# kvas7andy/unreal

Hardware: AMD Instinct MI355X
Metric: env-steps/sec (whole node), UNREAL maze 84x84 (higher is better)
Workload: dtype f32 (fp16x2-split MFMA operands, fp32 accumulate)

## Files before the change

unreal_amd/csrc/pc.hip:

```cpp
#include "common.h"

namespace {

constexpr int HP_LD = 36, HP_ROWS = 84;
constexpr int NPLP = 2;
constexpr int WD_ELEMS = 4 * 4 * 2 * 4 * 16 * 4;
constexpr int HP_V = (C2_POS * 8 + 255) / 256;
constexpr int DD_V = (PC_CELLS * 8 / 4 + 255) / 256;

struct PcFwdArgs {
  int N, A;
  const float* hp;
  const float* hp_absmax;
  const float* Wv; const float* bv; const float* Wa; const float* ba;
  float* qmax;
  const int* action;
  const float* target;
  const int* mask;
  float lambda, grad_scale;
  float* d_dec;
  float* ddec_absmax;
  float* loss;
};

__device__ __forceinline__ float deconv_w(const float* __restrict__ Wv, const float* __restrict__ Wa, int A, int ky, int kx,
                                          int co, int ci) {
  if (co == 0) return Wv[(ky * 4 + kx) * 32 + ci];
  if (co <= A) return Wa[((ky * 4 + kx) * A + (co - 1)) * 32 + ci];
  return 0.f;
}

__device__ __forceinline__ void hp_load(const float* __restrict__ src, int gtid, f32x4 (&r)[HP_V]) {
  const f32x4* s4 = reinterpret_cast<const f32x4*>(src);
#pragma unroll
  for (int c = 0; c < HP_V; ++c) {
    int id = gtid + 256 * c;
    r[c] = s4[id < C2_POS * 8 ? id : gtid];
  }
}

__device__ __forceinline__ void hp_store(float* hp, int gtid, const f32x4 (&r)[HP_V]) {
#pragma unroll
  for (int c = 0; c < HP_V; ++c) {
    int id = gtid + 256 * c;
    if (id < C2_POS * 8) *reinterpret_cast<f32x4*>(hp + (id >> 3) * HP_LD + (id & 7) * 4) = r[c];
  }
}

typedef _Float16 fh8p __attribute__((ext_vector_type(8)));
typedef _Float16 fh2p __attribute__((ext_vector_type(2)));
typedef float f32x2p __attribute__((ext_vector_type(2)));
typedef unsigned int u32x2p __attribute__((ext_vector_type(2)));

constexpr int HPP_ROW = 80;
constexpr int HPP_PLANE = HP_ROWS * HPP_ROW;
constexpr int WDP_ROW = 80;
constexpr int WDP_PLANE = 4 * 32 * WDP_ROW;

__device__ __forceinline__ void split4p(const f32x4& v, float scale, u32x2p (&pl)[NPLP]) {
  const f32x2p x01 = (f32x2p){v[0], v[1]} * scale, x23 = (f32x2p){v[2], v[3]} * scale;
  const fh2p h01 = __builtin_convertvector(x01, fh2p), h23 = __builtin_convertvector(x23, fh2p);
  const fh2p l01 = __builtin_convertvector(x01 - __builtin_convertvector(h01, f32x2p), fh2p);
  const fh2p l23 = __builtin_convertvector(x23 - __builtin_convertvector(h23, f32x2p), fh2p);
  pl[0] = (u32x2p){__builtin_bit_cast(unsigned int, h01), __builtin_bit_cast(unsigned int, h23)};
  pl[1] = (u32x2p){__builtin_bit_cast(unsigned int, l01), __builtin_bit_cast(unsigned int, l23)};
}

__device__ __forceinline__ void hp_store_planes(unsigned char* hpp, int gtid, const f32x4 (&r)[HP_V], float scale) {
#pragma unroll
  for (int c = 0; c < HP_V; ++c) {
    const int id = gtid + 256 * c;
    if (id < C2_POS * 8) {
      u32x2p pl[NPLP];
      split4p(r[c], scale, pl);
      pl[0][0] = keep_positive_visible(pl[0][0], r[c][0], r[c][1]);
      pl[0][1] = keep_positive_visible(pl[0][1], r[c][2], r[c][3]);
#pragma unroll
      for (int t = 0; t < NPLP; ++t) *reinterpret_cast<u32x2p*>(hpp + t * HPP_PLANE + (id >> 3) * HPP_ROW + (id & 7) * 8) = pl[t];
    }
  }
}

#define PC_MFMA(a, b, c) __builtin_amdgcn_mfma_f32_16x16x32_f16((a), (b), (c), 0, 0, 0)
#define PC_SPLIT_MMA(A, B, C)        \
  do {                               \
    C = PC_MFMA(A[1], B[0], C);      \
    C = PC_MFMA(A[0], B[1], C);      \
    C = PC_MFMA(A[0], B[0], C);      \
  } while (0)

__device__ __forceinline__ float pc_weight_max(const float* __restrict__ Wv, const float* __restrict__ Wa, int A, float* red) {
  if (threadIdx.x == 0) *red = 0.f;
  __syncthreads();
  float m = 0.f;
  for (int e = threadIdx.x; e < 512; e += 256) m = fmaxf(m, fabsf(Wv[e]));
  for (int e = threadIdx.x; e < 512 * A; e += 256) m = fmaxf(m, fabsf(Wa[e]));
  m = wave_max(m);
  if ((threadIdx.x & 63) == 0) atomicMax(reinterpret_cast<unsigned int*>(red), __float_as_uint(m));
  __syncthreads();
  return *red;
}

__device__ __forceinline__ void pc_fwd_weight_planes(const float* __restrict__ Wv, const float* __restrict__ Wa, int A,
                                                     unsigned char* wdp, float S_W) {
  const int CO = 1 + A;
  for (int e = threadIdx.x; e < 4 * 32 * 8; e += 256) {
    const int c4 = e & 7, n = (e >> 3) & 31, dd = e >> 8;
    f32x4 v = {0.f, 0.f, 0.f, 0.f};
    if (n < 4 * CO) {
      const int par = n / CO, co = n - par * CO;
      const int ky = (par >> 1) + 2 * (dd >> 1), kx = (par & 1) + 2 * (dd & 1);
#pragma unroll
      for (int k = 0; k < 4; ++k) v[k] = deconv_w(Wv, Wa, A, ky, kx, co, 4 * c4 + k);
    }
    u32x2p pl[NPLP];
    split4p(v, S_W, pl);
#pragma unroll
    for (int t = 0; t < NPLP; ++t) *reinterpret_cast<u32x2p*>(wdp + t * WDP_PLANE + (dd * 32 + n) * WDP_ROW + c4 * 8) = pl[t];
  }
}

__device__ __forceinline__ void pc_zero_hp_pad_rows(unsigned char* hpp) {
  for (int e = threadIdx.x; e < NPLP * 3 * HPP_ROW / 4; e += 256) {
    const int t = e / (3 * HPP_ROW / 4), w = e % (3 * HPP_ROW / 4);
    reinterpret_cast<uint32_t*>(hpp + t * HPP_PLANE + C2_POS * HPP_ROW)[w] = 0u;
  }
}

template <int COT> struct FwdLds {
  static constexpr int DS = COT | 1;
  static constexpr int DEC = NPLP * HPP_PLANE, DOUT = DEC + PC_CELLS * DS * 4, W = DOUT + PC_CELLS * COT * 4,
                       BYTES = W + NPLP * WDP_PLANE;
  static constexpr int WGS = 3 * BYTES <= 160 * 1024 ? 3 : 2;
};

template <bool TWO_NT, int DS>
__device__ __forceinline__ void deconv_packed(const unsigned char* hpp, const unsigned char* wdp, float* dec, int mt0, int i,
                                              int q, int CO, const float (&bias)[2], float unscale) {
  constexpr int NTL = TWO_NT ? 2 : 1;
  const int ntiles = (mt0 + 4 < 7) ? 2 : 1;
  f32x4 acc[2][NTL];
  int a[2], b[2];
#pragma unroll
  for (int t = 0; t < 2; ++t) {
#pragma unroll
    for (int nt = 0; nt < NTL; ++nt) acc[t][nt] = (f32x4){0.f, 0.f, 0.f, 0.f};
    const int m = min((mt0 + 4 * t) * 16 + i, 99);
    a[t] = m / 10;
    b[t] = m % 10;
  }
#pragma unroll
  for (int dd = 0; dd < 4; ++dd) {
    const int da = dd >> 1, db = dd & 1;
    fh8p bw[NTL][NPLP];
#pragma unroll
    for (int nt = 0; nt < NTL; ++nt)
#pragma unroll
      for (int pl = 0; pl < NPLP; ++pl)
        bw[nt][pl] = *reinterpret_cast<const fh8p*>(wdp + pl * WDP_PLANE + ((dd * 32 + nt * 16 + i)) * WDP_ROW + 16 * q);
#pragma unroll
    for (int t = 0; t < 2; ++t) {
      if (t < ntiles) {
        const int y = a[t] - da, x = b[t] - db;
        const int row = (y >= 0 && y < 9 && x >= 0 && x < 9) ? y * 9 + x : C2_POS;
        fh8p av[NPLP];
#pragma unroll
        for (int pl = 0; pl < NPLP; ++pl)
          av[pl] = *reinterpret_cast<const fh8p*>(hpp + pl * HPP_PLANE + row * HPP_ROW + 16 * q);
#pragma unroll
        for (int nt = 0; nt < NTL; ++nt) PC_SPLIT_MMA(av, bw[nt], acc[t][nt]);
      }
    }
  }
#pragma unroll
  for (int nt = 0; nt < NTL; ++nt) {
    const int n = nt * 16 + i;
    if (n < 4 * CO) {
      const int par = n / CO, co = n - par * CO;
#pragma unroll
      for (int t = 0; t < 2; ++t)
        if (t < ntiles) {
#pragma unroll
          for (int r = 0; r < 4; ++r) {
            const int m = (mt0 + 4 * t) * 16 + 4 * q + r;
            if (m < 100)
              dec[((2 * (m / 10) + (par >> 1)) * 20 + 2 * (m % 10) + (par & 1)) * DS + co] = acc[t][nt][r] * unscale + bias[nt];
          }
        }
    }
  }
}

template <int COT>
__global__ __launch_bounds__(256, FwdLds<COT>::WGS) void pc_deconv_fwd_kernel(PcFwdArgs p) {
  typedef FwdLds<COT> L;
  constexpr int DS = L::DS;
  __shared__ __attribute__((aligned(16))) unsigned char smem[L::BYTES];
  __shared__ float s_red;
  const int gtid = threadIdx.x;
  const int lane = threadIdx.x & 63, gw = gtid >> 6;
  const int i = lane & 15, q = lane >> 4;
  unsigned char* hpp = smem;
  float* dec = reinterpret_cast<float*>(smem + L::DEC);
  float* dout = reinterpret_cast<float*>(smem + L::DOUT);
  unsigned char* wdp = smem + L::W;
  const int A = p.A, CO = 1 + p.A;

  const float S_W = pow2_scale(pc_weight_max(p.Wv, p.Wa, A, &s_red));
  const float S_HP = pow2_scale(*p.hp_absmax);
  const float unscale = pow2_inv(S_HP) * pow2_inv(S_W);

  pc_fwd_weight_planes(p.Wv, p.Wa, A, wdp, S_W);
  pc_zero_hp_pad_rows(hpp);
  float bias[2];
#pragma unroll
  for (int nt = 0; nt < 2; ++nt) {
    const int n = nt * 16 + i;
    const int co = n % CO;
    bias[nt] = (n < 4 * CO) ? (co == 0 ? p.bv[0] : p.ba[co - 1]) : 0.f;
  }
  const bool two_nt = 4 * CO > 16;
  float loss_acc = 0.f, dd_max = 0.f;

  const int stride = gridDim.x;
  f32x4 pre[HP_V];
  {
    const int n0 = blockIdx.x;
    if (n0 < p.N) {
      hp_load(p.hp + (size_t)n0 * F2_DIM, gtid, pre);
      hp_store_planes(hpp, gtid, pre, S_HP);
    }
  }
  int prev = -1;
  for (int base = blockIdx.x; base < p.N; base += stride) {
    const int n = base;
    const bool valid = n < p.N;
    const int nn = n + stride;
    const bool has_next = nn < p.N;
    __syncthreads();
    if (prev >= 0 && p.d_dec) {
      f32x4* dst = reinterpret_cast<f32x4*>(p.d_dec + (size_t)prev * PC_CELLS * CO);
      for (int id = gtid; id < PC_CELLS * CO / 4; id += 256) dst[id] = reinterpret_cast<const f32x4*>(dout)[id];
    }
    if (has_next) hp_load(p.hp + (size_t)nn * F2_DIM, gtid, pre);
    float tg[2] = {0.f, 0.f};
    int act = 0;
    bool on = true;
    if (valid && p.d_dec) {
      tg[0] = p.target[(size_t)n * PC_CELLS + gtid];
      tg[1] = p.target[(size_t)n * PC_CELLS + min(gtid + 256, PC_CELLS - 1)];
      act = p.action[n];
      on = p.mask[n] != 0;
    }
    if (valid) {
      if (two_nt) deconv_packed<true, DS>(hpp, wdp, dec, gw, i, q, CO, bias, unscale);
      else deconv_packed<false, DS>(hpp, wdp, dec, gw, i, q, CO, bias, unscale);
    }
    __syncthreads();
    if (valid) {
#pragma unroll
      for (int pi = 0; pi < 2; ++pi) {
        const int pos = gtid + 256 * pi;
        if (pos >= PC_CELLS) break;
        const float* d = dec + pos * DS;
        const float vpre = d[0];
        const float V = fmaxf(vpre, 0.f);
        float adv[8], mean = 0.f;
        for (int k = 0; k < A; ++k) { adv[k] = fmaxf(d[1 + k], 0.f); mean += adv[k]; }
        mean /= (float)A;
        if (p.qmax) {
          float mx = V + adv[0] - mean;
          for (int k = 1; k < A; ++k) mx = fmaxf(mx, V + adv[k] - mean);
          p.qmax[(size_t)n * PC_CELLS + pos] = mx;
        }
        if (p.d_dec) {
          const float qa = V + adv[act] - mean;
          const float diff = tg[pi] - qa;
          const float dq = on ? -p.lambda * diff * p.grad_scale : 0.f;
          if (on) loss_acc += 0.5f * p.lambda * diff * diff;
          float* o = dout + pos * CO;
          o[0] = vpre > 0.f ? dq : 0.f;
          dd_max = fmaxf(dd_max, fabsf(dq));
          for (int k = 0; k < A; ++k)
            o[1 + k] = d[1 + k] > 0.f ? dq * (((k == act) ? 1.f : 0.f) - 1.f / (float)A) : 0.f;
        }
      }
    }
    if (has_next) hp_store_planes(hpp, gtid, pre, S_HP);
    prev = valid ? n : -1;
  }
  __syncthreads();
  if (prev >= 0 && p.d_dec) {
    f32x4* dst = reinterpret_cast<f32x4*>(p.d_dec + (size_t)prev * PC_CELLS * CO);
    for (int id = gtid; id < PC_CELLS * CO / 4; id += 256) dst[id] = reinterpret_cast<const f32x4*>(dout)[id];
  }
  {
    __shared__ float wsum[4], wmx[4];
    loss_acc = wave_sum(loss_acc);
    dd_max = wave_max(dd_max);
    if (lane == 0) { wsum[gw] = loss_acc; wmx[gw] = dd_max; }
    __syncthreads();
    if (gw == 0) {
      if (p.loss && lane == 0) atomicAdd(p.loss, (((wsum[0] + wsum[1]) + wsum[2]) + wsum[3]) * p.grad_scale);
      if (p.ddec_absmax) absmax_commit(p.ddec_absmax, fmaxf(fmaxf(wmx[0], wmx[1]), fmaxf(wmx[2], wmx[3])));
    }
  }
}

struct PcBwdArgs {
  int N, A;
  const float* hp;
  const float* hp_absmax;
  const float* d_dec;
  const float* ddec_absmax;
  const float* Wv; const float* Wa;
  float* d_hp;
  float* dWv; float* dbv; float* dWa; float* dba;
  float* dhp_absmax;
};

typedef short s16x4p __attribute__((ext_vector_type(4)));
typedef short s16x8p __attribute__((ext_vector_type(8)));
constexpr int DDP_ROW = 16;
constexpr int DDP_PLANE = (PC_CELLS + 4) * DDP_ROW;
constexpr int WBP_PLANE = 4 * 32 * WDP_ROW;
constexpr int BWD_GRP_BYTES = NPLP * HPP_PLANE + NPLP * DDP_PLANE + F2_DIM * 4;

__device__ __forceinline__ fh8p tr_pair_p(const unsigned char* a0, const unsigned char* a1) {
  typedef s16x4p __attribute__((address_space(3))) * lds_p;
  const s16x4p lo = __builtin_amdgcn_ds_read_tr16_b64_v4i16((lds_p)(a0));
  const s16x4p hi = __builtin_amdgcn_ds_read_tr16_b64_v4i16((lds_p)(a1));
  const s16x8p v = __builtin_shufflevector(lo, hi, 0, 1, 2, 3, 4, 5, 6, 7);
  return __builtin_bit_cast(fh8p, v);
}

__device__ __forceinline__ void split1p(float x, float scale, unsigned short (&t)[NPLP]) {
  x *= scale;
  const _Float16 h = (_Float16)x;
  const _Float16 l = (_Float16)(x - (float)h);
  t[0] = __builtin_bit_cast(unsigned short, h);
  t[1] = __builtin_bit_cast(unsigned short, l);
}

__device__ __forceinline__ void pc_bwd_weight_planes(const float* __restrict__ Wv, const float* __restrict__ Wa, int A,
                                                     unsigned char* wbp, float S_W) {
  for (int e = threadIdx.x; e < 4 * 32 * 32; e += 256) {
    const int k = e & 31, ci = (e >> 5) & 31, ky = e >> 10;
    const int kx = k >> 3, co = k & 7;
    float v = 0.f;
    if (co == 0) v = Wv[(ky * 4 + kx) * 32 + ci];
    else if (co <= A) v = Wa[((ky * 4 + kx) * A + (co - 1)) * 32 + ci];
    unsigned short t[NPLP];
    split1p(v, S_W, t);
#pragma unroll
    for (int pl = 0; pl < NPLP; ++pl)
      reinterpret_cast<unsigned short*>(wbp + pl * WBP_PLANE + (ky * 32 + ci) * WDP_ROW)[k] = t[pl];
  }
}

__device__ __forceinline__ void pc_stage_dd(unsigned char* ddp, int gtid, const float (&dd)[2][8], float S_DD, float (&adbk)[8]) {
#pragma unroll
  for (int h = 0; h < 2; ++h) {
    const int pos = gtid + 256 * h;
    if (pos < PC_CELLS) {
      u32x2p lo[NPLP], hi[NPLP];
      split4p((f32x4){dd[h][0], dd[h][1], dd[h][2], dd[h][3]}, S_DD, lo);
      split4p((f32x4){dd[h][4], dd[h][5], dd[h][6], dd[h][7]}, S_DD, hi);
#pragma unroll
      for (int pl = 0; pl < NPLP; ++pl) {
        typedef unsigned int u32x4p __attribute__((ext_vector_type(4)));
        *reinterpret_cast<u32x4p*>(ddp + pl * DDP_PLANE + pos * DDP_ROW) = (u32x4p){lo[pl][0], lo[pl][1], hi[pl][0], hi[pl][1]};
      }
#pragma unroll
      for (int k = 0; k < 8; ++k) adbk[k] += dd[h][k];
    }
  }
}

__device__ __forceinline__ void pc_dgrad_frame(const unsigned char* hpp, const unsigned char* ddp, const unsigned char* wbp,
                                               float* dhs, int gw, int i, int q, float un_dgrad) {
  const int nt = gw & 1;
  f32x4 acc[3];
  int abase[3];
#pragma unroll
  for (int jj = 0; jj < 3; ++jj) {
    acc[jj] = (f32x4){0.f, 0.f, 0.f, 0.f};
    const int pos = min(((gw >> 1) + 2 * jj) * 16 + i, C2_POS - 1);
    abase[jj] = ((2 * (pos / 9)) * 20 + 2 * (pos % 9) + q) * DDP_ROW;
  }
#pragma unroll
  for (int ky = 0; ky < 4; ++ky) {
    fh8p bw[NPLP];
#pragma unroll
    for (int pl = 0; pl < NPLP; ++pl)
      bw[pl] = *reinterpret_cast<const fh8p*>(wbp + pl * WBP_PLANE + (ky * 32 + nt * 16 + i) * WDP_ROW + 16 * q);
#pragma unroll
    for (int jj = 0; jj < 3; ++jj) {
      fh8p av[NPLP];
#pragma unroll
      for (int pl = 0; pl < NPLP; ++pl)
        av[pl] = *reinterpret_cast<const fh8p*>(ddp + pl * DDP_PLANE + abase[jj] + ky * 20 * DDP_ROW);
      PC_SPLIT_MMA(av, bw, acc[jj]);
    }
  }
#pragma unroll
  for (int jj = 0; jj < 3; ++jj)
#pragma unroll
    for (int r = 0; r < 4; ++r) {
      const int pos = ((gw >> 1) + 2 * jj) * 16 + 4 * q + r;
      if (pos < C2_POS) {
        const int ci = nt * 16 + i;
        const unsigned short h0 = reinterpret_cast<const unsigned short*>(hpp + pos * HPP_ROW)[ci];
        dhs[pos * 32 + ci] = (h0 != 0 && !(h0 & 0x8000)) ? acc[jj][r] * un_dgrad : 0.f;
      }
    }
}

__device__ __forceinline__ void pc_wgrad_frame(const unsigned char* hpp, const unsigned char* ddp, int gw, int i, int q,
                                               f32x4 (&aw)[2][2]) {
  const int qq = i >> 2, pp = i & 3;
#pragma unroll 1
  for (int ks = 0; ks < 3; ++ks) {
    const int p0 = 32 * ks + 8 * q + qq, p1 = p0 + 4;
    const unsigned char* b0 = hpp + min(p0, C2_POS) * HPP_ROW + 8 * pp;
    const unsigned char* b1 = hpp + min(p1, C2_POS) * HPP_ROW + 8 * pp;
    fh8p bf[2][NPLP];
#pragma unroll
    for (int t = 0; t < 2; ++t)
#pragma unroll
      for (int pl = 0; pl < NPLP; ++pl) bf[t][pl] = tr_pair_p(b0 + pl * HPP_PLANE + 32 * t, b1 + pl * HPP_PLANE + 32 * t);
    const int r0 = p0 < C2_POS ? (2 * (p0 / 9) + gw) * 20 + 2 * (p0 % 9) : PC_CELLS;
    const int r1 = p1 < C2_POS ? (2 * (p1 / 9) + gw) * 20 + 2 * (p1 % 9) : PC_CELLS;
#pragma unroll
    for (int kxh = 0; kxh < 2; ++kxh) {
      fh8p af[NPLP];
#pragma unroll
      for (int pl = 0; pl < NPLP; ++pl)
        af[pl] = tr_pair_p(ddp + pl * DDP_PLANE + (r0 + 2 * kxh) * DDP_ROW + 8 * pp,
                           ddp + pl * DDP_PLANE + (r1 + 2 * kxh) * DDP_ROW + 8 * pp);
      PC_SPLIT_MMA(af, bf[0], aw[kxh][0]);
      PC_SPLIT_MMA(af, bf[1], aw[kxh][1]);
    }
  }
}

__device__ __forceinline__ float pc_drain_dhp(const float* dhs, float* __restrict__ dst_frame, int gtid, float dhp_max) {
  f32x4* dst = reinterpret_cast<f32x4*>(dst_frame);
  for (int id = gtid; id < F2_DIM / 4; id += 256) {
    const f32x4 v = reinterpret_cast<const f32x4*>(dhs)[id];
    dst[id] = v;
    dhp_max = fmaxf(fmaxf(dhp_max, fmaxf(fabsf(v[0]), fabsf(v[1]))), fmaxf(fabsf(v[2]), fabsf(v[3])));
  }
  return dhp_max;
}

__device__ __forceinline__ void pc_commit_grads(const f32x4 (&aw)[2][2], float un_wgrad, const float (&adbk)[8], float dhp_max,
                                                int A, float* dWv, float* dWa, float* dbv, float* dba, float* dhp_absmax,
                                                float* red, int gw, int lane, int i, int q) {
  const int gtid = threadIdx.x, CO = 1 + A;
#pragma unroll
  for (int kxh = 0; kxh < 2; ++kxh)
#pragma unroll
    for (int t = 0; t < 2; ++t)
#pragma unroll
      for (int r = 0; r < 4; ++r) {
        int row = 4 * q + r;
        int kx = 2 * kxh + (row >> 3), co = row & 7, ci = t * 16 + i;
        float v = aw[kxh][t][r] * un_wgrad;
        if (co == 0) atomicAdd(dWv + (gw * 4 + kx) * 32 + ci, v);
        else if (co <= A) atomicAdd(dWa + ((gw * 4 + kx) * A + (co - 1)) * 32 + ci, v);
      }
  float* wsum = red;
  float* wmx = red + 32;
#pragma unroll
  for (int k = 0; k < 8; ++k) {
    const float v = wave_sum(adbk[k]);
    if (lane == 0) wsum[gw * 8 + k] = v;
  }
  dhp_max = wave_max(dhp_max);
  if (lane == 0) wmx[gw] = dhp_max;
  __syncthreads();
  if (gtid < CO) {
    const float v = ((wsum[gtid] + wsum[8 + gtid]) + wsum[16 + gtid]) + wsum[24 + gtid];
    if (gtid == 0) atomicAdd(dbv, v);
    else atomicAdd(dba + (gtid - 1), v);
  }
  if (gw == 0) absmax_commit(dhp_absmax, fmaxf(fmaxf(wmx[0], wmx[1]), fmaxf(wmx[2], wmx[3])));
}

__global__ __launch_bounds__(256, 2) void pc_deconv_bwd_kernel(PcBwdArgs p) {
  __shared__ __attribute__((aligned(16))) unsigned char smem[BWD_GRP_BYTES + NPLP * WBP_PLANE];
  __shared__ float s_red[36];
  static_assert(2 * (BWD_GRP_BYTES + NPLP * WBP_PLANE + 144) <= 160 * 1024, "two workgroups must fit one CU's LDS");
  const int gtid = threadIdx.x;
  const int lane = threadIdx.x & 63, gw = gtid >> 6;
  const int i = lane & 15, q = lane >> 4;
  unsigned char* hpp = smem;
  unsigned char* ddp = hpp + NPLP * HPP_PLANE;
  float* dhs = reinterpret_cast<float*>(ddp + NPLP * DDP_PLANE);
  unsigned char* wbp = smem + BWD_GRP_BYTES;
  const int A = p.A, CO = 1 + p.A;

  const float S_W = pow2_scale(pc_weight_max(p.Wv, p.Wa, A, s_red));
  const float S_HP = pow2_scale(*p.hp_absmax), S_DD = pow2_scale(*p.ddec_absmax);
  const float un_dgrad = pow2_inv(S_DD) * pow2_inv(S_W);
  const float un_wgrad = pow2_inv(S_DD) * pow2_inv(S_HP);

  pc_bwd_weight_planes(p.Wv, p.Wa, A, wbp, S_W);
  pc_zero_hp_pad_rows(hpp);
  for (int e = gtid; e < NPLP * DDP_PLANE / 4; e += 256) reinterpret_cast<uint32_t*>(ddp)[e] = 0u;

  f32x4 aw[2][2];
#pragma unroll
  for (int a = 0; a < 2; ++a)
#pragma unroll
    for (int b = 0; b < 2; ++b) aw[a][b] = (f32x4){0.f, 0.f, 0.f, 0.f};
  float adbk[8];
#pragma unroll
  for (int k = 0; k < 8; ++k) adbk[k] = 0.f;
  float dhp_max = 0.f;

  const int stride = gridDim.x;
  f32x4 pre_hp[HP_V];
  float pre_dd[2][8];
  auto load_dd = [&](int frame) {
    const float* src = p.d_dec + (size_t)frame * PC_CELLS * CO;
#pragma unroll
    for (int h = 0; h < 2; ++h) {
      const int pos = min(gtid + 256 * h, PC_CELLS - 1);
#pragma unroll
      for (int co = 0; co < 8; ++co) pre_dd[h][co] = (co < CO) ? src[pos * CO + co] : 0.f;
    }
  };

  __syncthreads();
  {
    const int n0 = blockIdx.x;
    if (n0 < p.N) {
      hp_load(p.hp + (size_t)n0 * F2_DIM, gtid, pre_hp);
      hp_store_planes(hpp, gtid, pre_hp, S_HP);
      load_dd(n0);
      pc_stage_dd(ddp, gtid, pre_dd, S_DD, adbk);
    }
  }
  for (int n = blockIdx.x; n < p.N; n += stride) {
    const int nn = n + stride;
    const bool has_next = nn < p.N;
    __syncthreads();
    if (has_next) {
      hp_load(p.hp + (size_t)nn * F2_DIM, gtid, pre_hp);
      load_dd(nn);
    }
    pc_dgrad_frame(hpp, ddp, wbp, dhs, gw, i, q, un_dgrad);
    pc_wgrad_frame(hpp, ddp, gw, i, q, aw);
    __syncthreads();
    dhp_max = pc_drain_dhp(dhs, p.d_hp + (size_t)n * F2_DIM, gtid, dhp_max);
    if (has_next) {
      hp_store_planes(hpp, gtid, pre_hp, S_HP);
      pc_stage_dd(ddp, gtid, pre_dd, S_DD, adbk);
    }
  }
  pc_commit_grads(aw, un_wgrad, adbk, dhp_max, A, p.dWv, p.dWa, p.dbv, p.dba, p.dhp_absmax, s_red, gw, lane, i, q);
}

struct PcTrainArgs {
  int N, A;
  const float* hp; const float* hp_absmax;
  const float* Wv; const float* bv; const float* Wa; const float* ba;
  const int* action; const float* target; const int* mask;
  float lambda, grad_scale;
  float* loss;
  float* d_hp; float* dhp_absmax;
  float* dWv; float* dbv; float* dWa; float* dba;
  float* d_dec;
};

template <int COT> struct TrainLds {
  static constexpr int DS = COT | 1;
  static constexpr int UNI = PC_CELLS * DS * 4 > F2_DIM * 4 ? PC_CELLS * DS * 4 : F2_DIM * 4;
  static constexpr int DDP = NPLP * HPP_PLANE, U = DDP + NPLP * DDP_PLANE, WF = U + UNI, WB = WF + NPLP * WDP_PLANE,
                       RED = WB + NPLP * WBP_PLANE, BYTES = RED + 192;
  static constexpr int WGS = 2 * BYTES <= 160 * 1024 ? 2 : 1;
};

template <int COT>
__global__ __launch_bounds__(256, TrainLds<COT>::WGS) void pc_deconv_train_kernel(PcTrainArgs p) {
  typedef TrainLds<COT> L;
  constexpr int DS = L::DS;
  __shared__ __attribute__((aligned(16))) unsigned char smem[L::BYTES];
  const int gtid = threadIdx.x;
  const int lane = threadIdx.x & 63, gw = gtid >> 6;
  const int i = lane & 15, q = lane >> 4;
  unsigned char* hpp = smem;
  unsigned char* ddp = smem + L::DDP;
  float* uni = reinterpret_cast<float*>(smem + L::U);
  unsigned char* wdp = smem + L::WF;
  unsigned char* wbp = smem + L::WB;
  float* red = reinterpret_cast<float*>(smem + L::RED);
  const int A = p.A, CO = 1 + p.A;

  const float S_W = pow2_scale(pc_weight_max(p.Wv, p.Wa, A, red));
  const float S_HP = pow2_scale(*p.hp_absmax);
  const float un_fwd = pow2_inv(S_HP) * pow2_inv(S_W);
  pc_fwd_weight_planes(p.Wv, p.Wa, A, wdp, S_W);
  pc_bwd_weight_planes(p.Wv, p.Wa, A, wbp, S_W);
  pc_zero_hp_pad_rows(hpp);
  for (int e = gtid; e < NPLP * DDP_PLANE / 4; e += 256) reinterpret_cast<uint32_t*>(ddp)[e] = 0u;
  float bias[2];
#pragma unroll
  for (int nt = 0; nt < 2; ++nt) {
    const int n = nt * 16 + i;
    const int co = n % CO;
    bias[nt] = (n < 4 * CO) ? (co == 0 ? p.bv[0] : p.ba[co - 1]) : 0.f;
  }
  const bool two_nt = 4 * CO > 16;

  f32x4 aw[2][2];
#pragma unroll
  for (int a = 0; a < 2; ++a)
#pragma unroll
    for (int b = 0; b < 2; ++b) aw[a][b] = (f32x4){0.f, 0.f, 0.f, 0.f};
  float adbk[8];
#pragma unroll
  for (int k = 0; k < 8; ++k) adbk[k] = 0.f;
  float dhp_max = 0.f, loss_acc = 0.f;

  const int stride = gridDim.x;
  f32x4 pre[HP_V];
  __syncthreads();
  if (blockIdx.x < p.N) {
    hp_load(p.hp + (size_t)blockIdx.x * F2_DIM, gtid, pre);
    hp_store_planes(hpp, gtid, pre, S_HP);
  }
  for (int n = blockIdx.x; n < p.N; n += stride) {
    const int nn = n + stride;
    const bool has_next = nn < p.N;
    __syncthreads();
    if (has_next) hp_load(p.hp + (size_t)nn * F2_DIM, gtid, pre);
    const float tg[2] = {p.target[(size_t)n * PC_CELLS + gtid], p.target[(size_t)n * PC_CELLS + min(gtid + 256, PC_CELLS - 1)]};
    const int act = p.action[n];
    const bool on = p.mask[n] != 0;
    if (two_nt) deconv_packed<true, DS>(hpp, wdp, uni, gw, i, q, CO, bias, un_fwd);
    else deconv_packed<false, DS>(hpp, wdp, uni, gw, i, q, CO, bias, un_fwd);
    __syncthreads();
    float dd[2][8];
    float fmx = 0.f;
#pragma unroll
    for (int pi = 0; pi < 2; ++pi) {
#pragma unroll
      for (int k = 0; k < 8; ++k) dd[pi][k] = 0.f;
      const int pos = gtid + 256 * pi;
      if (pos < PC_CELLS) {
        const float* d = uni + pos * DS;
        const float vpre = d[0];
        const float V = fmaxf(vpre, 0.f);
        float apre[COT - 1], mean = 0.f, aact = 0.f;
#pragma unroll
        for (int k = 0; k < COT - 1; ++k) {
          apre[k] = k < A ? d[1 + k] : 0.f;
          const float ad = fmaxf(apre[k], 0.f);
          mean += ad;
          aact = (k == act) ? ad : aact;
        }
        mean /= (float)A;
        const float qa = V + aact - mean;
        const float diff = tg[pi] - qa;
        const float dq = on ? -p.lambda * diff * p.grad_scale : 0.f;
        if (on) loss_acc += 0.5f * p.lambda * diff * diff;
        fmx = fmaxf(fmx, fabsf(dq));
        dd[pi][0] = vpre > 0.f ? dq : 0.f;
#pragma unroll
        for (int k = 0; k < COT - 1; ++k)
          dd[pi][1 + k] = (k < A && apre[k] > 0.f) ? dq * (((k == act) ? 1.f : 0.f) - 1.f / (float)A) : 0.f;
        if (p.d_dec) {
          float* o = p.d_dec + ((size_t)n * PC_CELLS + pos) * CO;
#pragma unroll
          for (int k = 0; k < COT; ++k)
            if (k < CO) o[k] = dd[pi][k];
        }
      }
    }
    fmx = wave_max(fmx);
    if (lane == 0) red[40 + gw] = fmx;
    __syncthreads();
    const float S_DD = pow2_scale(fmaxf(fmaxf(red[40], red[41]), fmaxf(red[42], red[43])));
    const float inv_dd = pow2_inv(S_DD);
    pc_stage_dd(ddp, gtid, dd, S_DD, adbk);
    __syncthreads();
    pc_dgrad_frame(hpp, ddp, wbp, uni, gw, i, q, inv_dd * pow2_inv(S_W));
    {
      f32x4 awf[2][2];
#pragma unroll
      for (int a = 0; a < 2; ++a)
#pragma unroll
        for (int b = 0; b < 2; ++b) awf[a][b] = (f32x4){0.f, 0.f, 0.f, 0.f};
      pc_wgrad_frame(hpp, ddp, gw, i, q, awf);
#pragma unroll
      for (int a = 0; a < 2; ++a)
#pragma unroll
        for (int b = 0; b < 2; ++b) aw[a][b] += awf[a][b] * inv_dd;
    }
    __syncthreads();
    dhp_max = pc_drain_dhp(uni, p.d_hp + (size_t)n * F2_DIM, gtid, dhp_max);
    if (has_next) hp_store_planes(hpp, gtid, pre, S_HP);
  }
  __syncthreads();
  loss_acc = wave_sum(loss_acc);
  if (lane == 0) red[44 + gw] = loss_acc;
  pc_commit_grads(aw, pow2_inv(S_HP), adbk, dhp_max, A, p.dWv, p.dWa, p.dbv, p.dba, p.dhp_absmax, red, gw, lane, i, q);
  if (gtid == 0) atomicAdd(p.loss, (((red[44] + red[45]) + red[46]) + red[47]) * p.grad_scale);
}

constexpr int WIDE_CO = UNREAL_MAX_ACTIONS + 1;
constexpr int WIDE_HS_LD = 33;
constexpr int WIDE_HS_BYTES = 82 * WIDE_HS_LD * 4;
constexpr int WIDE_WT_LD = 32 * WIDE_CO;
constexpr int WIDE_WS_BYTES = 16 * WIDE_WT_LD * 4;
constexpr int WIDE_DD_BYTES = PC_CELLS * WIDE_CO * 4;
constexpr int WIDE_WG_ENTRIES = (16 * WIDE_CO + 7) / 8;
constexpr int WIDE_FWD_BYTES = WIDE_HS_BYTES + WIDE_WS_BYTES;
constexpr int WIDE_TRAIN_BYTES = WIDE_FWD_BYTES + WIDE_DD_BYTES;
static_assert(3 * (WIDE_FWD_BYTES + 64) <= 160 * 1024, "three wide forward workgroups must fit one CU's LDS");
static_assert(2 * (WIDE_TRAIN_BYTES + 192) <= 160 * 1024, "two wide training workgroups must fit one CU's LDS");

__device__ __forceinline__ void wide_stage_weights(const float* __restrict__ Wv, const float* __restrict__ Wa, int A,
                                                   float* ws) {
  for (int e = threadIdx.x; e < 16 * 32 * WIDE_CO; e += 256) {
    const int co = e % WIDE_CO, ci = (e / WIDE_CO) & 31, tap = e / (32 * WIDE_CO);
    float v = 0.f;
    if (co == 0) v = Wv[tap * 32 + ci];
    else if (co <= A) v = Wa[(tap * A + (co - 1)) * 32 + ci];
    ws[e] = v;
  }
}

__device__ __forceinline__ void wide_stage_hp(const float* __restrict__ src, float* hs) {
  const f32x4* s4 = reinterpret_cast<const f32x4*>(src);
  for (int id = threadIdx.x; id < C2_POS * 8; id += 256) {
    const f32x4 v = s4[id];
    float* d = hs + (id >> 3) * WIDE_HS_LD + (id & 7) * 4;
    d[0] = v[0]; d[1] = v[1]; d[2] = v[2]; d[3] = v[3];
  }
}

__device__ __forceinline__ int wide_deconv_slot(const float* hs, const float* ws, int s, int CO,
                                                const float (&bias)[WIDE_CO], float (&out)[WIDE_CO]) {
  const int par = s / 100, m = s - 100 * par, a = m / 10, b = m - 10 * (m / 10);
  const int pa = par >> 1, pb = par & 1;
#pragma unroll
// ... 363 lines not shown
```

Before: 3.784 million.

## Swizzle LDS planes, precompute address tables, and software-pipeline PC MFMA loops

Shrinks the fp16 plane row pitch from 80 to 64 bytes and applies an XOR swizzle so LDS reads stay bank-conflict free with less LDS per workgroup. Per-lane LDS offsets for the deconv, dgrad and wgrad loops are computed once into packed 16-bit tables instead of per frame. The MFMA loops are double-buffered with explicit sched_group_barrier interleaving of LDS reads and MFMAs. Out-of-range stores are redirected to a dump region so the epilogue has no branches. Also hard-codes the action count from the template when possible and re-pitches the dd staging buffer. The risks are higher register pressure from the tables and double buffers, and layout changes that must stay consistent across every reader.

```diff
diff --git a/unreal_amd/csrc/pc.hip b/unreal_amd/csrc/pc.hip
--- a/unreal_amd/csrc/pc.hip
+++ b/unreal_amd/csrc/pc.hip
@@ -52,10 +52,24 @@
 typedef float f32x2p __attribute__((ext_vector_type(2)));
 typedef unsigned int u32x2p __attribute__((ext_vector_type(2)));
 
-constexpr int HPP_ROW = 80;
+constexpr int HPP_ROW = 64;
 constexpr int HPP_PLANE = HP_ROWS * HPP_ROW;
-constexpr int WDP_ROW = 80;
+constexpr int WDP_ROW = 64;
 constexpr int WDP_PLANE = 4 * 32 * WDP_ROW;
+__device__ __forceinline__ int hpp_off(int row, int b) { return row * HPP_ROW + (b ^ ((((row >> 2) ^ (row >> 3)) & 1) << 5)); }
+__device__ __forceinline__ int wrow_off(int row, int b) { return row * WDP_ROW + (b ^ (((row >> 3) & 1) << 5)); }
+
+#define LO16(x) ((x) & 0xffffu)
+#define HI16(x) ((x) >> 16)
+#define PIN(x) asm volatile("" : "+v"(x))
+template <int N, int NV, int ND> __device__ __forceinline__ void pc_interleave() {
+#pragma unroll
+  for (int k = 0; k < N; ++k) {
+    __builtin_amdgcn_sched_group_barrier(0x008, 1, 0);
+    __builtin_amdgcn_sched_group_barrier(0x002, NV, 0);
+    __builtin_amdgcn_sched_group_barrier(0x080, ND, 0);
+  }
+}
 
 __device__ __forceinline__ void split4p(const f32x4& v, float scale, u32x2p (&pl)[NPLP]) {
   const f32x2p x01 = (f32x2p){v[0], v[1]} * scale, x23 = (f32x2p){v[2], v[3]} * scale;
@@ -76,7 +90,7 @@
       pl[0][0] = keep_positive_visible(pl[0][0], r[c][0], r[c][1]);
       pl[0][1] = keep_positive_visible(pl[0][1], r[c][2], r[c][3]);
 #pragma unroll
-      for (int t = 0; t < NPLP; ++t) *reinterpret_cast<u32x2p*>(hpp + t * HPP_PLANE + (id >> 3) * HPP_ROW + (id & 7) * 8) = pl[t];
+      for (int t = 0; t < NPLP; ++t) *reinterpret_cast<u32x2p*>(hpp + t * HPP_PLANE + hpp_off(id >> 3, (id & 7) * 8)) = pl[t];
     }
   }
 }
@@ -116,7 +130,7 @@
     u32x2p pl[NPLP];
     split4p(v, S_W, pl);
 #pragma unroll
-    for (int t = 0; t < NPLP; ++t) *reinterpret_cast<u32x2p*>(wdp + t * WDP_PLANE + (dd * 32 + n) * WDP_ROW + c4 * 8) = pl[t];
+    for (int t = 0; t < NPLP; ++t) *reinterpret_cast<u32x2p*>(wdp + t * WDP_PLANE + wrow_off(dd * 32 + n, c4 * 8)) = pl[t];
   }
 }
 
@@ -127,68 +141,110 @@
   }
 }
 
+constexpr int DEC_DUMP = 32 * 4;
 template <int COT> struct FwdLds {
   static constexpr int DS = COT | 1;
-  static constexpr int DEC = NPLP * HPP_PLANE, DOUT = DEC + PC_CELLS * DS * 4, W = DOUT + PC_CELLS * COT * 4,
+  static constexpr int DEC = NPLP * HPP_PLANE, DOUT = DEC + PC_CELLS * DS * 4 + DEC_DUMP, W = DOUT + PC_CELLS * COT * 4,
                        BYTES = W + NPLP * WDP_PLANE;
-  static constexpr int WGS = 3 * BYTES <= 160 * 1024 ? 3 : 2;
+  static constexpr int WGS = COT <= 5 ? 3 : 2;
+  static_assert(WGS * (BYTES + 64) <= 160 * 1024, "the forward workgroups of one CU must fit its LDS");
 };
 
-template <bool TWO_NT, int DS>
-__device__ __forceinline__ void deconv_packed(const unsigned char* hpp, const unsigned char* wdp, float* dec, int mt0, int i,
-                                              int q, int CO, const float (&bias)[2], float unscale) {
+struct PcFwdTab {
+  uint32_t a[4];
+  uint32_t w;
+  uint32_t dst[2][2][2];
+};
+
+template <int DS>
+__device__ __forceinline__ void pc_fwd_tab_build(PcFwdTab& T, int mt0, int lane, int CO) {
+  const int i = lane & 15, q = lane >> 4;
+  uint32_t o[4][2];
+#pragma unroll
+  for (int t = 0; t < 2; ++t) {
+    const int m = min((mt0 + 4 * t) * 16 + i, 99);
+    const int a = m / 10, b = m % 10;
+#pragma unroll
+    for (int dd = 0; dd < 4; ++dd) {
+      const int y = a - (dd >> 1), x = b - (dd & 1);
+      const int row = (y >= 0 && y < 9 && x >= 0 && x < 9) ? y * 9 + x : C2_POS;
+      o[dd][t] = hpp_off(row, 16 * q);
+    }
+  }
+#pragma unroll
+  for (int dd = 0; dd < 4; ++dd) T.a[dd] = o[dd][0] | (o[dd][1] << 16);
+  T.w = wrow_off(i, 16 * q);
+  const uint32_t dump = PC_CELLS * DS * 4 + (lane & 31) * 4;
+#pragma unroll
+  for (int t = 0; t < 2; ++t)
+#pragma unroll
+    for (int nt = 0; nt < 2; ++nt) {
+      const int n = nt * 16 + i;
+      const int par = n / CO, co = n - par * CO;
+      uint32_t d[4];
+#pragma unroll
+      for (int r = 0; r < 4; ++r) {
+        const int m = (mt0 + 4 * t) * 16 + 4 * q + r;
+        d[r] = (n < 4 * CO && m < 100) ? (uint32_t)(((2 * (m / 10) + (par >> 1)) * 20 + 2 * (m % 10) + (par & 1)) * DS + co) * 4 : dump;
+      }
+      T.dst[t][nt][0] = d[0] | (d[1] << 16);
+      T.dst[t][nt][1] = d[2] | (d[3] << 16);
+    }
+}
+
+template <bool TWO_NT, int NTILES>
+__device__ __forceinline__ void deconv_packed(const unsigned char* hpp, const unsigned char* wdp, float* dec, PcFwdTab& T,
+                                              const float (&bias)[2], float unscale) {
   constexpr int NTL = TWO_NT ? 2 : 1;
-  const int ntiles = (mt0 + 4 < 7) ? 2 : 1;
-  f32x4 acc[2][NTL];
-  int a[2], b[2];
-#pragma unroll
-  for (int t = 0; t < 2; ++t) {
+  f32x4 acc[NTILES][NTL];
+#pragma unroll
+  for (int t = 0; t < NTILES; ++t)
 #pragma unroll
     for (int nt = 0; nt < NTL; ++nt) acc[t][nt] = (f32x4){0.f, 0.f, 0.f, 0.f};
-    const int m = min((mt0 + 4 * t) * 16 + i, 99);
-    a[t] = m / 10;
-    b[t] = m % 10;
-  }
+  fh8p bw[2][NTL][NPLP], av[2][NTILES][NPLP];
+  PIN(T.w);
+  auto load = [&](int dd) {
+    PIN(T.a[dd]);
+#pragma unroll
+    for (int nt = 0; nt < NTL; ++nt)
+#pragma unroll
+      for (int pl = 0; pl < NPLP; ++pl)
+        bw[dd & 1][nt][pl] = *reinterpret_cast<const fh8p*>(wdp + pl * WDP_PLANE + (dd * 32 + nt * 16) * WDP_ROW + T.w);
+#pragma unroll
+    for (int t = 0; t < NTILES; ++t) {
+      const unsigned char* ap = hpp + (t ? HI16(T.a[dd]) : LO16(T.a[dd]));
+#pragma unroll
+      for (int pl = 0; pl < NPLP; ++pl) av[dd & 1][t][pl] = *reinterpret_cast<const fh8p*>(ap + pl * HPP_PLANE);
+    }
+  };
+  load(0);
 #pragma unroll
   for (int dd = 0; dd < 4; ++dd) {
-    const int da = dd >> 1, db = dd & 1;
-    fh8p bw[NTL][NPLP];
+    if (dd + 1 < 4) load(dd + 1);
+#pragma unroll
+    for (int t = 0; t < NTILES; ++t)
+#pragma unroll
+      for (int nt = 0; nt < NTL; ++nt) PC_SPLIT_MMA(av[dd & 1][t], bw[dd & 1][nt], acc[t][nt]);
+    pc_interleave<3 * NTILES * NTL, 1, 1>();
+    __builtin_amdgcn_sched_barrier(0);
+  }
+#pragma unroll
+  for (int t = 0; t < NTILES; ++t)
 #pragma unroll
     for (int nt = 0; nt < NTL; ++nt)
 #pragma unroll
-      for (int pl = 0; pl < NPLP; ++pl)
-        bw[nt][pl] = *reinterpret_cast<const fh8p*>(wdp + pl * WDP_PLANE + ((dd * 32 + nt * 16 + i)) * WDP_ROW + 16 * q);
-#pragma unroll
-    for (int t = 0; t < 2; ++t) {
-      if (t < ntiles) {
-        const int y = a[t] - da, x = b[t] - db;
-        const int row = (y >= 0 && y < 9 && x >= 0 && x < 9) ? y * 9 + x : C2_POS;
-        fh8p av[NPLP];
-#pragma unroll
-        for (int pl = 0; pl < NPLP; ++pl)
-          av[pl] = *reinterpret_cast<const fh8p*>(hpp + pl * HPP_PLANE + row * HPP_ROW + 16 * q);
-#pragma unroll
-        for (int nt = 0; nt < NTL; ++nt) PC_SPLIT_MMA(av, bw[nt], acc[t][nt]);
+      for (int r = 0; r < 4; ++r) {
+        if (!(r & 1)) PIN(T.dst[t][nt][r >> 1]);
+        const uint32_t o = (r & 1) ? HI16(T.dst[t][nt][r >> 1]) : LO16(T.dst[t][nt][r >> 1]);
+        *reinterpret_cast<float*>(reinterpret_cast<unsigned char*>(dec) + o) = acc[t][nt][r] * unscale + bias[nt];
       }
-    }
-  }
-#pragma unroll
-  for (int nt = 0; nt < NTL; ++nt) {
-    const int n = nt * 16 + i;
-    if (n < 4 * CO) {
-      const int par = n / CO, co = n - par * CO;
-#pragma unroll
-      for (int t = 0; t < 2; ++t)
-        if (t < ntiles) {
-#pragma unroll
-          for (int r = 0; r < 4; ++r) {
-            const int m = (mt0 + 4 * t) * 16 + 4 * q + r;
-            if (m < 100)
-              dec[((2 * (m / 10) + (par >> 1)) * 20 + 2 * (m % 10) + (par & 1)) * DS + co] = acc[t][nt][r] * unscale + bias[nt];
-          }
-        }
-    }
-  }
+}
+
+template <bool TWO_NT>
+__device__ __forceinline__ void deconv_packed_wave(const unsigned char* hpp, const unsigned char* wdp, float* dec, PcFwdTab& T,
+                                                   int gw, const float (&bias)[2], float unscale) {
+  if (gw + 4 < 7) deconv_packed<TWO_NT, 2>(hpp, wdp, dec, T, bias, unscale);
+  else deconv_packed<TWO_NT, 1>(hpp, wdp, dec, T, bias, unscale);
 }
 
 template <int COT>
@@ -198,13 +254,13 @@
   __shared__ __attribute__((aligned(16))) unsigned char smem[L::BYTES];
   __shared__ float s_red;
   const int gtid = threadIdx.x;
-  const int lane = threadIdx.x & 63, gw = gtid >> 6;
-  const int i = lane & 15, q = lane >> 4;
+  const int lane = threadIdx.x & 63, gw = __builtin_amdgcn_readfirstlane(gtid >> 6);
+  const int i = lane & 15;
   unsigned char* hpp = smem;
   float* dec = reinterpret_cast<float*>(smem + L::DEC);
   float* dout = reinterpret_cast<float*>(smem + L::DOUT);
   unsigned char* wdp = smem + L::W;
-  const int A = p.A, CO = 1 + p.A;
+  const int A = COT < 8 ? COT - 1 : p.A, CO = 1 + A;
 
   const float S_W = pow2_scale(pc_weight_max(p.Wv, p.Wa, A, &s_red));
   const float S_HP = pow2_scale(*p.hp_absmax);
@@ -219,7 +275,9 @@
     const int co = n % CO;
     bias[nt] = (n < 4 * CO) ? (co == 0 ? p.bv[0] : p.ba[co - 1]) : 0.f;
   }
-  const bool two_nt = 4 * CO > 16;
+  constexpr bool TWO_NT = 4 * COT > 16;
+  PcFwdTab T;
+  pc_fwd_tab_build<DS>(T, gw, lane, CO);
   float loss_acc = 0.f, dd_max = 0.f;
 
   const int stride = gridDim.x;
@@ -253,8 +311,7 @@
       on = p.mask[n] != 0;
     }
     if (valid) {
-      if (two_nt) deconv_packed<true, DS>(hpp, wdp, dec, gw, i, q, CO, bias, unscale);
-      else deconv_packed<false, DS>(hpp, wdp, dec, gw, i, q, CO, bias, unscale);
+      deconv_packed_wave<TWO_NT>(hpp, wdp, dec, T, gw, bias, unscale);
     }
     __syncthreads();
     if (valid) {
@@ -322,9 +379,12 @@
 typedef short s16x4p __attribute__((ext_vector_type(4)));
 typedef short s16x8p __attribute__((ext_vector_type(8)));
 constexpr int DDP_ROW = 16;
-constexpr int DDP_PLANE = (PC_CELLS + 4) * DDP_ROW;
+constexpr int DDP_PITCH = 25;
+constexpr int DDP_ZERO = 20 * DDP_PITCH;
+constexpr int DDP_PLANE = (DDP_ZERO + 5) * DDP_ROW;
 constexpr int WBP_PLANE = 4 * 32 * WDP_ROW;
-constexpr int BWD_GRP_BYTES = NPLP * HPP_PLANE + NPLP * DDP_PLANE + F2_DIM * 4;
+constexpr int DHS_BYTES = (C2_POS + 4) * 128;
+constexpr int BWD_GRP_BYTES = NPLP * HPP_PLANE + NPLP * DDP_PLANE + DHS_BYTES;
 
 __device__ __forceinline__ fh8p tr_pair_p(const unsigned char* a0, const unsigned char* a1) {
   typedef s16x4p __attribute__((address_space(3))) * lds_p;
@@ -354,93 +414,151 @@
     split1p(v, S_W, t);
 #pragma unroll
     for (int pl = 0; pl < NPLP; ++pl)
-      reinterpret_cast<unsigned short*>(wbp + pl * WBP_PLANE + (ky * 32 + ci) * WDP_ROW)[k] = t[pl];
-  }
-}
-
-__device__ __forceinline__ void pc_stage_dd(unsigned char* ddp, int gtid, const float (&dd)[2][8], float S_DD, float (&adbk)[8]) {
-#pragma unroll
-  for (int h = 0; h < 2; ++h) {
-    const int pos = gtid + 256 * h;
-    if (pos < PC_CELLS) {
-      u32x2p lo[NPLP], hi[NPLP];
-      split4p((f32x4){dd[h][0], dd[h][1], dd[h][2], dd[h][3]}, S_DD, lo);
-      split4p((f32x4){dd[h][4], dd[h][5], dd[h][6], dd[h][7]}, S_DD, hi);
-#pragma unroll
-      for (int pl = 0; pl < NPLP; ++pl) {
-        typedef unsigned int u32x4p __attribute__((ext_vector_type(4)));
-        *reinterpret_cast<u32x4p*>(ddp + pl * DDP_PLANE + pos * DDP_ROW) = (u32x4p){lo[pl][0], lo[pl][1], hi[pl][0], hi[pl][1]};
-      }
-#pragma unroll
-      for (int k = 0; k < 8; ++k) adbk[k] += dd[h][k];
-    }
-  }
-}
-
-__device__ __forceinline__ void pc_dgrad_frame(const unsigned char* hpp, const unsigned char* ddp, const unsigned char* wbp,
-                                               float* dhs, int gw, int i, int q, float un_dgrad) {
-  const int nt = gw & 1;
-  f32x4 acc[3];
-  int abase[3];
+      *reinterpret_cast<unsigned short*>(wbp + pl * WBP_PLANE + wrow_off(ky * 32 + ci, 2 * k)) = t[pl];
+  }
+}
+
+struct PcBwdTab {
+  uint32_t st;
+  uint32_t da[2];
+  uint32_t dw;
+  uint32_t de[3];
+  uint32_t wb[3][2];
+  uint32_t wa[3];
+};
+
+__device__ __forceinline__ int ddp_row(int pos) { return (pos / 20) * DDP_PITCH + pos % 20; }
+
+__device__ __forceinline__ void pc_bwd_tab_build(PcBwdTab& T, int gtid, int gw) {
+  const int lane = gtid & 63, i = lane & 15, q = lane >> 4, nt = gw & 1;
+  const int qq = i >> 2, pp = i & 3;
+  {
+    const uint32_t s0 = ddp_row(gtid) * DDP_ROW;
+    const uint32_t s1 = (gtid + 256 < PC_CELLS ? ddp_row(gtid + 256) : DDP_ZERO + 4) * DDP_ROW;
+    T.st = s0 | (s1 << 16);
+  }
+  uint32_t ab[3];
 #pragma unroll
   for (int jj = 0; jj < 3; ++jj) {
-    acc[jj] = (f32x4){0.f, 0.f, 0.f, 0.f};
-    const int pos = min(((gw >> 1) + 2 * jj) * 16 + i, C2_POS - 1);
-    abase[jj] = ((2 * (pos / 9)) * 20 + 2 * (pos % 9) + q) * DDP_ROW;
-  }
-#pragma unroll
-  for (int ky = 0; ky < 4; ++ky) {
-    fh8p bw[NPLP];
-#pragma unroll
-    for (int pl = 0; pl < NPLP; ++pl)
-      bw[pl] = *reinterpret_cast<const fh8p*>(wbp + pl * WBP_PLANE + (ky * 32 + nt * 16 + i) * WDP_ROW + 16 * q);
-#pragma unroll
-    for (int jj = 0; jj < 3; ++jj) {
-      fh8p av[NPLP];
-#pragma unroll
-      for (int pl = 0; pl < NPLP; ++pl)
-        av[pl] = *reinterpret_cast<const fh8p*>(ddp + pl * DDP_PLANE + abase[jj] + ky * 20 * DDP_ROW);
-      PC_SPLIT_MMA(av, bw, acc[jj]);
-    }
-  }
-#pragma unroll
-  for (int jj = 0; jj < 3; ++jj)
-#pragma unroll
-    for (int r = 0; r < 4; ++r) {
-      const int pos = ((gw >> 1) + 2 * jj) * 16 + 4 * q + r;
-      if (pos < C2_POS) {
-        const int ci = nt * 16 + i;
-        const unsigned short h0 = reinterpret_cast<const unsigned short*>(hpp + pos * HPP_ROW)[ci];
-        dhs[pos * 32 + ci] = (h0 != 0 && !(h0 & 0x8000)) ? acc[jj][r] * un_dgrad : 0.f;
-      }
-    }
-}
-
-__device__ __forceinline__ void pc_wgrad_frame(const unsigned char* hpp, const unsigned char* ddp, int gw, int i, int q,
-                                               f32x4 (&aw)[2][2]) {
-  const int qq = i >> 2, pp = i & 3;
-#pragma unroll 1
+    const int tile = (gw >> 1) + 2 * jj;
+    const int pos = min(tile * 16 + i, C2_POS - 1);
+    ab[jj] = ((2 * (pos / 9)) * DDP_PITCH + 2 * (pos % 9) + q) * DDP_ROW;
+    const int p0 = tile * 16 + 4 * q, ci = nt * 16 + i;
+    const bool live = p0 < C2_POS;
+    T.de[jj] = (uint32_t)hpp_off(live ? p0 : C2_POS - 1, 2 * ci) | ((uint32_t)((live ? p0 : C2_POS) * 128 + ci * 4) << 16);
+  }
+  T.da[0] = ab[0] | (ab[1] << 16);
+  T.da[1] = ab[2];
+  T.dw = wrow_off(nt * 16 + i, 16 * q);
+#pragma unroll
   for (int ks = 0; ks < 3; ++ks) {
     const int p0 = 32 * ks + 8 * q + qq, p1 = p0 + 4;
-    const unsigned char* b0 = hpp + min(p0, C2_POS) * HPP_ROW + 8 * pp;
-    const unsigned char* b1 = hpp + min(p1, C2_POS) * HPP_ROW + 8 * pp;
-    fh8p bf[2][NPLP];
 #pragma unroll
     for (int t = 0; t < 2; ++t)
-#pragma unroll
-      for (int pl = 0; pl < NPLP; ++pl) bf[t][pl] = tr_pair_p(b0 + pl * HPP_PLANE + 32 * t, b1 + pl * HPP_PLANE + 32 * t);
-    const int r0 = p0 < C2_POS ? (2 * (p0 / 9) + gw) * 20 + 2 * (p0 % 9) : PC_CELLS;
-    const int r1 = p1 < C2_POS ? (2 * (p1 / 9) + gw) * 20 + 2 * (p1 % 9) : PC_CELLS;
-#pragma unroll
-    for (int kxh = 0; kxh < 2; ++kxh) {
-      fh8p af[NPLP];
-#pragma unroll
-      for (int pl = 0; pl < NPLP; ++pl)
-        af[pl] = tr_pair_p(ddp + pl * DDP_PLANE + (r0 + 2 * kxh) * DDP_ROW + 8 * pp,
-                           ddp + pl * DDP_PLANE + (r1 + 2 * kxh) * DDP_ROW + 8 * pp);
-      PC_SPLIT_MMA(af, bf[0], aw[kxh][0]);
-      PC_SPLIT_MMA(af, bf[1], aw[kxh][1]);
-    }
+      T.wb[ks][t] = (uint32_t)hpp_off(min(p0, C2_POS), 8 * pp + 32 * t) | ((uint32_t)hpp_off(min(p1, C2_POS), 8 * pp + 32 * t) << 16);
+    const int r0 = p0 < C2_POS ? (2 * (p0 / 9) + gw) * DDP_PITCH + 2 * (p0 % 9) : DDP_ZERO;
+    const int r1 = p1 < C2_POS ? (2 * (p1 / 9) + gw) * DDP_PITCH + 2 * (p1 % 9) : DDP_ZERO;
+    T.wa[ks] = (uint32_t)(r0 * DDP_ROW + 8 * pp) | ((uint32_t)(r1 * DDP_ROW + 8 * pp) << 16);
+  }
+}
+
+__device__ __forceinline__ void pc_stage_dd(unsigned char* ddp, PcBwdTab& T, const float (&dd)[2][8], float S_DD, float (&adbk)[8]) {
+  PIN(T.st);
+#pragma unroll
+  for (int h = 0; h < 2; ++h) {
+    unsigned char* row = ddp + (h ? HI16(T.st) : LO16(T.st));
+    u32x2p lo[NPLP], hi[NPLP];
+    split4p((f32x4){dd[h][0], dd[h][1], dd[h][2], dd[h][3]}, S_DD, lo);
+    split4p((f32x4){dd[h][4], dd[h][5], dd[h][6], dd[h][7]}, S_DD, hi);
+#pragma unroll
+    for (int pl = 0; pl < NPLP; ++pl) {
+      typedef unsigned int u32x4p __attribute__((ext_vector_type(4)));
+      *reinterpret_cast<u32x4p*>(row + pl * DDP_PLANE) = (u32x4p){lo[pl][0], lo[pl][1], hi[pl][0], hi[pl][1]};
+    }
+#pragma unroll
+    for (int k = 0; k < 8; ++k) adbk[k] += dd[h][k];
+  }
+}
+
+__device__ __forceinline__ void pc_dgrad_frame(const unsigned char* hpp, const unsigned char* ddp, const unsigned char* wbp,
+                                               float* dhs, PcBwdTab& T, float un_dgrad) {
+  f32x4 acc[3];
+  fh8p bw[4][NPLP], av[2][NPLP];
+  PIN(T.dw);
+  PIN(T.da[0]);
+  PIN(T.da[1]);
+  auto load_av = [&](int s) {
+    const int jj = s >> 2, ky = s & 3;
+    const unsigned char* ap = ddp + (jj == 0 ? LO16(T.da[0]) : jj == 1 ? HI16(T.da[0]) : T.da[1]) + ky * DDP_PITCH * DDP_ROW;
+#pragma unroll
+    for (int pl = 0; pl < NPLP; ++pl) av[s & 1][pl] = *reinterpret_cast<const fh8p*>(ap + pl * DDP_PLANE);
+  };
+  auto epilogue = [&](int jj) {
+    PIN(T.de[jj]);
+    const unsigned char* hrow = hpp + LO16(T.de[jj]);
+    unsigned char* drow = reinterpret_cast<unsigned char*>(dhs) + HI16(T.de[jj]);
+#pragma unroll
+    for (int r = 0; r < 4; ++r) {
+      const unsigned short h0 = *reinterpret_cast<const unsigned short*>(hrow + r * HPP_ROW);
+      *reinterpret_cast<float*>(drow + r * 128) = (h0 != 0 && !(h0 & 0x8000)) ? acc[jj][r] * un_dgrad : 0.f;
+    }
+  };
+#pragma unroll
+  for (int ky = 0; ky < 4; ++ky)
+#pragma unroll
+    for (int pl = 0; pl < NPLP; ++pl)
+      bw[ky][pl] = *reinterpret_cast<const fh8p*>(wbp + pl * WBP_PLANE + ky * 32 * WDP_ROW + T.dw);
+  load_av(0);
+#pragma unroll
+  for (int s = 0; s < 12; ++s) {
+    const int jj = s >> 2, ky = s & 3;
+    if (ky == 0) acc[jj] = (f32x4){0.f, 0.f, 0.f, 0.f};
+    if (s + 1 < 12) load_av(s + 1);
+    PC_SPLIT_MMA(av[s & 1], bw[ky], acc[jj]);
+    if (ky == 0 && jj > 0) {
+      epilogue(jj - 1);
+      pc_interleave<3, 6, 4>();
+    } else {
+      pc_interleave<3, 1, 1>();
+    }
+    __builtin_amdgcn_sched_barrier(0);
+  }
+  epilogue(2);
+}
+
+__device__ __forceinline__ void pc_wgrad_frame(const unsigned char* hpp, const unsigned char* ddp, PcBwdTab& T, f32x4 (&aw)[2][2]) {
+  fh8p bf[2][2][NPLP];
+  fh8p af[2][NPLP];
+  auto load_bf = [&](int ks) {
+#pragma unroll
+    for (int t = 0; t < 2; ++t) {
+      PIN(T.wb[ks][t]);
+      const unsigned char* b0 = hpp + LO16(T.wb[ks][t]);
+      const unsigned char* b1 = hpp + HI16(T.wb[ks][t]);
+#pragma unroll
+      for (int pl = 0; pl < NPLP; ++pl) bf[ks & 1][t][pl] = tr_pair_p(b0 + pl * HPP_PLANE, b1 + pl * HPP_PLANE);
+    }
+  };
+  auto load_af = [&](int s) {
+    const int ks = s >> 1, kxh = s & 1;
+    if (kxh == 0) PIN(T.wa[ks]);
+    const unsigned char* a0 = ddp + LO16(T.wa[ks]) + 2 * kxh * DDP_ROW;
+    const unsigned char* a1 = ddp + HI16(T.wa[ks]) + 2 * kxh * DDP_ROW;
+#pragma unroll
+    for (int pl = 0; pl < NPLP; ++pl) af[s & 1][pl] = tr_pair_p(a0 + pl * DDP_PLANE, a1 + pl * DDP_PLANE);
+  };
+  load_bf(0);
+  load_af(0);
+#pragma unroll
+  for (int s = 0; s < 6; ++s) {
+    const int ks = s >> 1, kxh = s & 1;
+    if (s + 1 < 6) load_af(s + 1);
+    if (kxh == 0 && ks + 1 < 3) load_bf(ks + 1);
+    PC_SPLIT_MMA(af[s & 1], bf[ks & 1][0], aw[kxh][0]);
+    PC_SPLIT_MMA(af[s & 1], bf[ks & 1][1], aw[kxh][1]);
+    if (kxh == 0 && ks + 1 < 3) pc_interleave<6, 1, 2>();
+    else pc_interleave<6, 1, 1>();
+    __builtin_amdgcn_sched_barrier(0);
   }
 }
 
@@ -508,6 +626,8 @@
 
   pc_bwd_weight_planes(p.Wv, p.Wa, A, wbp, S_W);
   pc_zero_hp_pad_rows(hpp);
+  PcBwdTab T;
+  pc_bwd_tab_build(T, gtid, gw);
   for (int e = gtid; e < NPLP * DDP_PLANE / 4; e += 256) reinterpret_cast<uint32_t*>(ddp)[e] = 0u;
 
   f32x4 aw[2][2];
@@ -527,9 +647,9 @@
     const float* src = p.d_dec + (size_t)frame * PC_CELLS * CO;
 #pragma unroll
     for (int h = 0; h < 2; ++h) {
-      const int pos = min(gtid + 256 * h, PC_CELLS - 1);
-#pragma unroll
-      for (int co = 0; co < 8; ++co) pre_dd[h][co] = (co < CO) ? src[pos * CO + co] : 0.f;
+      const int pos = gtid + 256 * h;
+#pragma unroll
+      for (int co = 0; co < 8; ++co) pre_dd[h][co] = (co < CO && pos < PC_CELLS) ? src[pos * CO + co] : 0.f;
     }
   };
 
@@ -540,7 +660,7 @@
       hp_load(p.hp + (size_t)n0 * F2_DIM, gtid, pre_hp);
       hp_store_planes(hpp, gtid, pre_hp, S_HP);
       load_dd(n0);
-      pc_stage_dd(ddp, gtid, pre_dd, S_DD, adbk);
+      pc_stage_dd(ddp, T, pre_dd, S_DD, adbk);
     }
   }
   for (int n = blockIdx.x; n < p.N; n += stride) {
@@ -551,13 +671,13 @@
       hp_load(p.hp + (size_t)nn * F2_DIM, gtid, pre_hp);
       load_dd(nn);
     }
-    pc_dgrad_frame(hpp, ddp, wbp, dhs, gw, i, q, un_dgrad);
-    pc_wgrad_frame(hpp, ddp, gw, i, q, aw);
+    pc_dgrad_frame(hpp, ddp, wbp, dhs, T, un_dgrad);
+    pc_wgrad_frame(hpp, ddp, T, aw);
     __syncthreads();
     dhp_max = pc_drain_dhp(dhs, p.d_hp + (size_t)n * F2_DIM, gtid, dhp_max);
     if (has_next) {
       hp_store_planes(hpp, gtid, pre_hp, S_HP);
-      pc_stage_dd(ddp, gtid, pre_dd, S_DD, adbk);
+      pc_stage_dd(ddp, T, pre_dd, S_DD, adbk);
     }
   }
   pc_commit_grads(aw, un_wgrad, adbk, dhp_max, A, p.dWv, p.dWa, p.dbv, p.dba, p.dhp_absmax, s_red, gw, lane, i, q);
@@ -577,10 +697,11 @@
 
 template <int COT> struct TrainLds {
   static constexpr int DS = COT | 1;
-  static constexpr int UNI = PC_CELLS * DS * 4 > F2_DIM * 4 ? PC_CELLS * DS * 4 : F2_DIM * 4;
+  static constexpr int UNI = PC_CELLS * DS * 4 + DEC_DUMP > DHS_BYTES ? PC_CELLS * DS * 4 + DEC_DUMP : DHS_BYTES;
   static constexpr int DDP = NPLP * HPP_PLANE, U = DDP + NPLP * DDP_PLANE, WF = U + UNI, WB = WF + NPLP * WDP_PLANE,
                        RED = WB + NPLP * WBP_PLANE, BYTES = RED + 192;
-  static constexpr int WGS = 2 * BYTES <= 160 * 1024 ? 2 : 1;
+  static constexpr int WGS = 2;
+  static_assert(2 * BYTES <= 160 * 1024, "two training workgroups must fit one CU's LDS");
 };
 
 template <int COT>
@@ -589,7 +710,7 @@
   constexpr int DS = L::DS;
   __shared__ __attribute__((aligned(16))) unsigned char smem[L::BYTES];
   const int gtid = threadIdx.x;
-  const int lane = threadIdx.x & 63, gw = gtid >> 6;
+  const int lane = threadIdx.x & 63, gw = __builtin_amdgcn_readfirstlane(gtid >> 6);
   const int i = lane & 15, q = lane >> 4;
   unsigned char* hpp = smem;
   unsigned char* ddp = smem + L::DDP;
@@ -597,7 +718,7 @@
   unsigned char* wdp = smem + L::WF;
   unsigned char* wbp = smem + L::WB;
   float* red = reinterpret_cast<float*>(smem + L::RED);
-  const int A = p.A, CO = 1 + p.A;
+  const int A = COT < 8 ? COT - 1 : p.A, CO = 1 + A;
 
   const float S_W = pow2_scale(pc_weight_max(p.Wv, p.Wa, A, red));
   const float S_HP = pow2_scale(*p.hp_absmax);
@@ -613,7 +734,11 @@
     const int co = n % CO;
     bias[nt] = (n < 4 * CO) ? (co == 0 ? p.bv[0] : p.ba[co - 1]) : 0.f;
   }
-  const bool two_nt = 4 * CO > 16;
+  constexpr bool TWO_NT = 4 * COT > 16;
+  PcFwdTab TF;
+  pc_fwd_tab_build<DS>(TF, gw, lane, CO);
+  PcBwdTab TB;
+  pc_bwd_tab_build(TB, gtid, gw);
 
   f32x4 aw[2][2];
 #pragma unroll
@@ -640,8 +765,7 @@
     const float tg[2] = {p.target[(size_t)n * PC_CELLS + gtid], p.target[(size_t)n * PC_CELLS + min(gtid + 256, PC_CELLS - 1)]};
     const int act = p.action[n];
     const bool on = p.mask[n] != 0;
-    if (two_nt) deconv_packed<true, DS>(hpp, wdp, uni, gw, i, q, CO, bias, un_fwd);
-    else deconv_packed<false, DS>(hpp, wdp, uni, gw, i, q, CO, bias, un_fwd);
+    deconv_packed_wave<TWO_NT>(hpp, wdp, uni, TF, gw, bias, un_fwd);
     __syncthreads();
     float dd[2][8];
     float fmx = 0.f;
@@ -685,16 +809,16 @@
     __syncthreads();
     const float S_DD = pow2_scale(fmaxf(fmaxf(red[40], red[41]), fmaxf(red[42], red[43])));
     const float inv_dd = pow2_inv(S_DD);
-    pc_stage_dd(ddp, gtid, dd, S_DD, adbk);
-    __syncthreads();
-    pc_dgrad_frame(hpp, ddp, wbp, uni, gw, i, q, inv_dd * pow2_inv(S_W));
+    pc_stage_dd(ddp, TB, dd, S_DD, adbk);
+    __syncthreads();
+    pc_dgrad_frame(hpp, ddp, wbp, uni, TB, inv_dd * pow2_inv(S_W));
     {
       f32x4 awf[2][2];
 #pragma unroll
       for (int a = 0; a < 2; ++a)
 #pragma unroll
         for (int b = 0; b < 2; ++b) awf[a][b] = (f32x4){0.f, 0.f, 0.f, 0.f};
-      pc_wgrad_frame(hpp, ddp, gw, i, q, awf);
+      pc_wgrad_frame(hpp, ddp, TB, awf);
 #pragma unroll
       for (int a = 0; a < 2; ++a)
 #pragma unroll
```

After: 3.836 million, median of 6. +1.4%, better.
